# sMedX/FaceNet

Hardware: AMD Instinct MI355X
Metric: images/sec (160x160 triplet train) (higher is better)
Workload: dtype bf16

## Files before the change

facenet_amd/csrc/block_fused.hip:

```cpp
#include "common.h"
#include "../../include/facenet_hip.h"
#include <cstdlib>

namespace fn {

struct Block17Args {
    const unsigned short* x;
    unsigned short* y;
    const unsigned short* w_t0;
    const unsigned short* w_t1a;
    const unsigned short* w_t1b;
    const unsigned short* w_t1c;
    const unsigned short* w_up;
    const float* b_t0;
    const float* b_t1a;
    const float* b_t1b;
    const float* b_t1c;
    const float* b_up;
    float scale;
    int relu;
    int N;
    const unsigned char* warm;
    long warm_bytes;
};

enum { WARM_WGS = 64 };
__device__ __forceinline__ void warm_range(const unsigned char* p, long bytes, int j, int nthreads) {
    const long per = ((bytes + 8 * 16 - 1) / (8 * 16)) * 16;
    const long lo = (long)(j >> 3) * per, hi = lo + per < bytes ? lo + per : bytes;
    unsigned acc = 0u;
    for (long o = lo + (long)threadIdx.x * 16; o + 16 <= hi; o += (long)nthreads * 16 * 4) {
        u32x4 v[4];
#pragma unroll
        for (int u = 0; u < 4; ++u) {
            const long oo = o + (long)u * nthreads * 16;
            v[u] = oo + 16 <= hi ? *reinterpret_cast<const u32x4*>(p + oo) : u32x4{0u, 0u, 0u, 0u};
        }
#pragma unroll
        for (int u = 0; u < 4; ++u) acc ^= v[u][0];
    }
    asm volatile("" ::"v"(acc));
}

__device__ __forceinline__ int swz64(int row, int chunk) { return row * 64 + ((chunk ^ (((row >> 2) & 1) << 1)) << 4); }

#define FN_RING_PIPELINE(D_, NT_, LOAD, STORE, COMPUTE)                                   \
    {                                                                                       \
        _Pragma("unroll") for (int d_ = 0; d_ < (D_); ++d_) { LOAD(min(d_, (NT_) - 1), d_) } \
        STORE(0, 0)                                                                         \
        LOAD(min((D_), (NT_) - 1), 0)                                                       \
        __syncthreads();                                                                    \
        for (int kt0_ = 0; kt0_ < (NT_); kt0_ += (D_)) {                                    \
            _Pragma("unroll") for (int d_ = 0; d_ < (D_); ++d_) {                           \
                const int kt_ = kt0_ + d_;                                                  \
                if (kt_ < (NT_)) {                                                          \
                    STORE((d_ + 1) & 1, (d_ + 1) % (D_))                                    \
                    LOAD(min(kt_ + 1 + (D_), (NT_) - 1), (d_ + 1) % (D_))                   \
                    COMPUTE(kt_, d_ & 1, d_)                                                \
                    __syncthreads();                                                        \
                }                                                                           \
            }                                                                               \
        }                                                                                   \
    }

#define FN_DMA_PIPELINE(U_, NT_, ISSUE, COMPUTE)                                          \
    {                                                                                       \
        ISSUE(0, 0)                                                                         \
        ISSUE(min(1, (NT_) - 1), 1)                                                         \
        for (int kt0_ = 0; kt0_ < (NT_); kt0_ += (U_)) {                                    \
            _Pragma("unroll") for (int d_ = 0; d_ < (U_); ++d_) {                           \
                const int kt_ = kt0_ + d_;                                                  \
                if (kt_ < (NT_)) {                                                          \
                    asm volatile("s_waitcnt vmcnt(2)" ::: "memory");    \
                    __builtin_amdgcn_s_barrier();                       \
                    ISSUE(min(kt_ + 2, (NT_) - 1), (d_ + 2) % 3)                            \
                    COMPUTE(kt_, d_ % 3, d_)                                                \
                }                                                                           \
            }                                                                               \
        }                                                                                   \
        asm volatile("s_waitcnt vmcnt(0)" ::: "memory");                                    \
        __builtin_amdgcn_s_barrier();                                                       \
    }

template <typename T, bool DMA>
__global__ __launch_bounds__(512) void block17_infer_kernel(const Block17Args a) {
    constexpr int C = 896, CT = 128, NPIX = 64, D = 4;
    constexpr int DMA_BUF = 16 * 1024;
    typedef __attribute__((address_space(3))) void* lds_ptr;
    constexpr int PATCH_PIX = 112;
    constexpr int MIXED_BYTES = 8 * NPIX * 64;
    constexpr int PATCH_BYTES = 4 * PATCH_PIX * 64;
    constexpr int STAGE_BYTES = 20 * 1024;
    typedef typename LP<T>::vec8 vec8;

    extern __shared__ __attribute__((aligned(16))) unsigned char smem[];
    unsigned char* sMixed = smem;
    unsigned char* sT1a = sMixed + MIXED_BYTES;
    unsigned char* sT1b = sT1a + PATCH_BYTES;
    unsigned char* sStage = sT1b + PATCH_BYTES;
    float* sC = reinterpret_cast<float*>(sT1a);

    const int tid = threadIdx.x, lane = tid & 63, wave = tid >> 6, wq = wave & 3, wh = wave >> 2;
    const int fr = lane & 15, fq = lane >> 4;
    const int img = blockIdx.x;
    if (img >= a.N) {
        warm_range(a.warm, a.warm_bytes, img - a.N, 512);
        return;
    }
    const unsigned short* xin = a.x + (long)img * NPIX * C;
    const __amdgpu_buffer_rsrc_t rs_x = __builtin_amdgcn_make_buffer_rsrc(const_cast<unsigned short*>(xin), 0, NPIX * C * 2, 0x00020000);

    for (int i = tid; i < 2 * PATCH_BYTES / 16; i += 512) reinterpret_cast<u32x4*>(sT1a)[i] = u32x4{0u, 0u, 0u, 0u};

    {
        const int lrow = tid >> 2, lch = tid & 3;
        const __amdgpu_buffer_rsrc_t rs_w0 = __builtin_amdgcn_make_buffer_rsrc(const_cast<unsigned short*>(a.w_t0), 0, CT * C * 2, 0x00020000);
        const __amdgpu_buffer_rsrc_t rs_w1 = __builtin_amdgcn_make_buffer_rsrc(const_cast<unsigned short*>(a.w_t1a), 0, CT * C * 2, 0x00020000);
        f32x4 acc[2][4];
#pragma unroll
        for (int i = 0; i < 2; ++i)
#pragma unroll
            for (int j = 0; j < 4; ++j) acc[i][j] = f32x4{0.f, 0.f, 0.f, 0.f};
        u32x4 ra[D], rb[D][2];
        const int voff = (lrow * C + lch * 8) * 2;
        const int voff_x = ((lrow & 63) * C + lch * 8) * 2;
        const int st_a = swz64(lrow & 63, lch);
        int st_b[2], fa_off[2], fb_off[4];
#pragma unroll
        for (int q = 0; q < 2; ++q) st_b[q] = 4096 + swz64(lrow + 128 * q, lch);
#pragma unroll
        for (int i = 0; i < 2; ++i) fa_off[i] = swz64(wh * 32 + i * 16 + fr, fq);
#pragma unroll
        for (int j = 0; j < 4; ++j) fb_off[j] = 4096 + swz64(wq * 64 + j * 16 + fr, fq);
#define S1_LOAD(kt, d)                                                                                    \
        ra[d] = __builtin_amdgcn_raw_buffer_load_b128(rs_x, voff_x, (kt) * 64, 0);                         \
        rb[d][0] = __builtin_amdgcn_raw_buffer_load_b128(rs_w0, voff, (kt) * 64, 0);                       \
        rb[d][1] = __builtin_amdgcn_raw_buffer_load_b128(rs_w1, voff, (kt) * 64, 0);
#define S1_STORE(buf, d)                                                                                   \
        if (wh == 0) *reinterpret_cast<u32x4*>(sStage + (buf) * STAGE_BYTES + st_a) = ra[d];                 \
        _Pragma("unroll") for (int q = 0; q < 2; ++q) *reinterpret_cast<u32x4*>(sStage + (buf) * STAGE_BYTES + st_b[q]) = rb[d][q];
#define S1_COMPUTE(kt, buf, d)                                                                                           \
        {                                                                                                                  \
            vec8 fa[2], fb[4];                                                                                             \
            _Pragma("unroll") for (int i = 0; i < 2; ++i) fa[i] = *reinterpret_cast<const vec8*>(sStage + (buf) * STAGE_BYTES + fa_off[i]); \
            _Pragma("unroll") for (int j = 0; j < 4; ++j) fb[j] = *reinterpret_cast<const vec8*>(sStage + (buf) * STAGE_BYTES + fb_off[j]); \
            _Pragma("unroll") for (int i = 0; i < 2; ++i)                                                                  \
                _Pragma("unroll") for (int j = 0; j < 4; ++j) acc[i][j] = LP<T>::mfma(fa[i], fb[j], acc[i][j]);            \
        }
        FN_RING_PIPELINE(D, C / 32, S1_LOAD, S1_STORE, S1_COMPUTE)
#undef S1_LOAD
#undef S1_STORE
#undef S1_COMPUTE
#pragma unroll
        for (int j = 0; j < 4; ++j) {
            const int col = (wq & 1) * 64 + j * 16 + fr;
            const float bias = wq < 2 ? a.b_t0[col] : a.b_t1a[col];
            const int slice = col >> 5, cc = col & 31;
#pragma unroll
            for (int i = 0; i < 2; ++i)
#pragma unroll
                for (int r = 0; r < 4; ++r) {
                    const int p = wh * 32 + i * 16 + fq * 4 + r;
                    const unsigned short h = LP<T>::from_f32(fmaxf(acc[i][j][r] + bias, 0.f));
                    if (wq < 2) {
                        *reinterpret_cast<unsigned short*>(sMixed + slice * (NPIX * 64) + swz64(p, cc >> 3) + (cc & 7) * 2) = h;
                    } else {
                        const int pidx = (p >> 3) * 14 + (p & 7) + 3;
                        *reinterpret_cast<unsigned short*>(sT1a + slice * (PATCH_PIX * 64) + swz64(pidx, cc >> 3) + (cc & 7) * 2) = h;
                    }
                }
        }
        __syncthreads();
    }

    const int srow = tid >> 3, sch = tid & 7;
    int sl_off[2], fb_off[2][2];
#pragma unroll
    for (int q = 0; q < 2; ++q) sl_off[q] = (srow + 64 * q) * 128 + ((sch ^ ((srow + 64 * q) & 7)) << 4);
#pragma unroll
    for (int h = 0; h < 2; ++h)
#pragma unroll
        for (int j = 0; j < 2; ++j) {
            const int rw = wq * 32 + j * 16 + fr;
            fb_off[h][j] = rw * 128 + (((h * 4 + fq) ^ (rw & 7)) << 4);
        }
#define SLAB_STORE(buf, d) \
        _Pragma("unroll") for (int q = 0; q < 2; ++q) *reinterpret_cast<u32x4*>(sStage + (buf) * STAGE_BYTES + sl_off[q]) = rb[d][q];

#pragma unroll 1
    for (int stage = 2; stage <= 3; ++stage) {
        const unsigned short* wgt = stage == 2 ? a.w_t1b : a.w_t1c;
        const __amdgpu_buffer_rsrc_t rs_w = __builtin_amdgcn_make_buffer_rsrc(const_cast<unsigned short*>(wgt), 0, CT * 7 * CT * 2, 0x00020000);
        const float* bias_p = stage == 2 ? a.b_t1b : a.b_t1c;
        const unsigned char* src = stage == 2 ? sT1a : sT1b;
        const int tstep = stage == 2 ? 1 : 8;
        f32x4 acc[2][2];
#pragma unroll
        for (int i = 0; i < 2; ++i)
#pragma unroll
            for (int j = 0; j < 2; ++j) acc[i][j] = f32x4{0.f, 0.f, 0.f, 0.f};
        int fa_off[7][2];
#pragma unroll
        for (int t = 0; t < 7; ++t)
#pragma unroll
            for (int i = 0; i < 2; ++i) {
                const int p = wh * 32 + i * 16 + fr;
                const int base = stage == 2 ? (p >> 3) * 14 + (p & 7) : p;
                fa_off[t][i] = swz64(base + t * tstep, fq);
            }
        u32x4 rb[D][2];
        const int voff = (srow * (7 * CT) + sch * 8) * 2;
#define S23_LOAD(kt, d)                                                                                                         \
        _Pragma("unroll") for (int q = 0; q < 2; ++q)                                                                            \
            rb[d][q] = __builtin_amdgcn_raw_buffer_load_b128(rs_w, voff + 64 * q * (7 * CT) * 2, (((kt) >> 1) * CT + ((kt) & 1) * 64) * 2, 0);
#define S23_TAP(TAP, buf, half)                                                                                                  \
        _Pragma("unroll") for (int h = 0; h < 2; ++h) {                                                                          \
            vec8 fa[2], fb[2];                                                                                                   \
            _Pragma("unroll") for (int i = 0; i < 2; ++i)                                                                        \
                fa[i] = *reinterpret_cast<const vec8*>(src + ((half) * 2 + h) * (PATCH_PIX * 64) + fa_off[TAP][i]);              \
            _Pragma("unroll") for (int j = 0; j < 2; ++j) fb[j] = *reinterpret_cast<const vec8*>(sStage + (buf) * STAGE_BYTES + fb_off[h][j]); \
            _Pragma("unroll") for (int i = 0; i < 2; ++i)                                                                        \
                _Pragma("unroll") for (int j = 0; j < 2; ++j) acc[i][j] = LP<T>::mfma(fa[i], fb[j], acc[i][j]);                  \
        }
#define S23_COMPUTE(kt, buf, d)                                                                                                  \
        {                                                                                                                        \
            const int g = (kt) >> 2;                             \
            if ((d) < 2) {                                                                                                       \
                if (g == 0) { S23_TAP(0, buf, (d) & 1) } else if (g == 1) { S23_TAP(2, buf, (d) & 1) }                           \
                else if (g == 2) { S23_TAP(4, buf, (d) & 1) } else { S23_TAP(6, buf, (d) & 1) }                                  \
            } else {                                                                                                             \
                if (g == 0) { S23_TAP(1, buf, (d) & 1) } else if (g == 1) { S23_TAP(3, buf, (d) & 1) } else { S23_TAP(5, buf, (d) & 1) } \
            }                                                                                                                    \
        }
        if constexpr (DMA) {
#define S23_DMA_ISSUE(kt, buf)                                                                                               \
            _Pragma("unroll") for (int q = 0; q < 2; ++q)                                                                        \
                __builtin_amdgcn_raw_ptr_buffer_load_lds(rs_w, (lds_ptr)(sStage + (buf) * DMA_BUF + (wave * 16 + 8 * q) * 128), 16,   \
                                                         dma_voff23[q], (((kt) >> 1) * CT + ((kt) & 1) * 64) * 2, 0, 0);
#define S23_DMA_FB(buf, h, j) *reinterpret_cast<const vec8*>(sStage + (buf) * DMA_BUF + fb_off[h][j])
#define S23_DMA_TAP(TAP, buf, half)                                                                                              \
            _Pragma("unroll") for (int h = 0; h < 2; ++h) {                                                                      \
                vec8 fa[2], fb[2];                                                                                               \
                _Pragma("unroll") for (int i = 0; i < 2; ++i)                                                                    \
                    fa[i] = *reinterpret_cast<const vec8*>(src + ((half) * 2 + h) * (PATCH_PIX * 64) + fa_off[TAP][i]);          \
                _Pragma("unroll") for (int j = 0; j < 2; ++j) fb[j] = S23_DMA_FB(buf, h, j);                                     \
                _Pragma("unroll") for (int i = 0; i < 2; ++i)                                                                    \
                    _Pragma("unroll") for (int j = 0; j < 2; ++j) acc[i][j] = LP<T>::mfma(fa[i], fb[j], acc[i][j]);              \
            }
#define S23_DMA_COMPUTE(kt, buf, d)                                                                                              \
            {                                                                                                                    \
                const int g = (kt) / 6;                                                                             \
                if (((d) >> 1) == 0) { if (g == 0) { S23_DMA_TAP(0, buf, (d) & 1) } else if (g == 1) { S23_DMA_TAP(3, buf, (d) & 1) } else { S23_DMA_TAP(6, buf, (d) & 1) } } \
                else if (((d) >> 1) == 1) { if (g == 0) { S23_DMA_TAP(1, buf, (d) & 1) } else { S23_DMA_TAP(4, buf, (d) & 1) } } \
                else { if (g == 0) { S23_DMA_TAP(2, buf, (d) & 1) } else { S23_DMA_TAP(5, buf, (d) & 1) } }                      \
            }
            int dma_voff23[2];
#pragma unroll
            for (int q = 0; q < 2; ++q) {
                const int r = wave * 16 + 8 * q + (lane >> 3), cs = (lane & 7) ^ (r & 7);
                dma_voff23[q] = (r * (7 * CT) + cs * 8) * 2;
            }
            FN_DMA_PIPELINE(6, 14, S23_DMA_ISSUE, S23_DMA_COMPUTE)
#undef S23_DMA_ISSUE
#undef S23_DMA_FB
#undef S23_DMA_TAP
#undef S23_DMA_COMPUTE
        } else {
            FN_RING_PIPELINE(D, 14, S23_LOAD, SLAB_STORE, S23_COMPUTE)
        }
#undef S23_LOAD
#undef S23_TAP
#undef S23_COMPUTE
#pragma unroll
        for (int j = 0; j < 2; ++j) {
            const int col = wq * 32 + j * 16 + fr;
            const float bias = bias_p[col];
            const int slice = col >> 5, cc = col & 31;
#pragma unroll
            for (int i = 0; i < 2; ++i)
#pragma unroll
                for (int r = 0; r < 4; ++r) {
                    const int p = wh * 32 + i * 16 + fq * 4 + r;
                    const unsigned short h = LP<T>::from_f32(fmaxf(acc[i][j][r] + bias, 0.f));
                    if (stage == 2) *reinterpret_cast<unsigned short*>(sT1b + slice * (PATCH_PIX * 64) + swz64(p + 24, cc >> 3) + (cc & 7) * 2) = h;
                    else *reinterpret_cast<unsigned short*>(sMixed + (4 + slice) * (NPIX * 64) + swz64(p, cc >> 3) + (cc & 7) * 2) = h;
                }
        }
        __syncthreads();
    }

    {
        constexpr int CLD = 132;
        const __amdgpu_buffer_rsrc_t rs_w = __builtin_amdgcn_make_buffer_rsrc(const_cast<unsigned short*>(a.w_up), 0, C * 256 * 2, 0x00020000);
        u32x4 rb[D][2];
        const int voff = (srow * 256 + sch * 8) * 2;
        int fa_off[2];
#pragma unroll
        for (int i = 0; i < 2; ++i) fa_off[i] = swz64(wh * 32 + i * 16 + fr, fq);
        f32x4 acc[2][2];
#define S4_LOAD(kt, d)                                                                                                           \
        _Pragma("unroll") for (int q = 0; q < 2; ++q)                                                                            \
            rb[d][q] = __builtin_amdgcn_raw_buffer_load_b128(rs_w, voff + 64 * q * 256 * 2, ((((kt) >> 2) * 128) * 256 + ((kt) & 3) * 64) * 2, 0);
#define S4_COMPUTE(kt, buf, d)                                                                                                   \
        {                                                                                                                        \
            if ((d) == 0) {                                                                                                      \
                _Pragma("unroll") for (int i = 0; i < 2; ++i)                                                                    \
                    _Pragma("unroll") for (int j = 0; j < 2; ++j) acc[i][j] = f32x4{0.f, 0.f, 0.f, 0.f};                         \
            }                                                                                                                    \
            _Pragma("unroll") for (int h = 0; h < 2; ++h) {                                                                      \
                vec8 fa[2], fb[2];                                                                                               \
                _Pragma("unroll") for (int i = 0; i < 2; ++i)                                                                    \
                    fa[i] = *reinterpret_cast<const vec8*>(sMixed + ((d) * 2 + h) * (NPIX * 64) + fa_off[i]);                    \
                _Pragma("unroll") for (int j = 0; j < 2; ++j) fb[j] = *reinterpret_cast<const vec8*>(sStage + (buf) * STAGE_BYTES + fb_off[h][j]); \
                _Pragma("unroll") for (int i = 0; i < 2; ++i)                                                                    \
                    _Pragma("unroll") for (int j = 0; j < 2; ++j) acc[i][j] = LP<T>::mfma(fa[i], fb[j], acc[i][j]);              \
            }                                                                                                                    \
            if ((d) == 3) {                 \
                const int pass = (kt) >> 2;                                                                                      \
                _Pragma("unroll") for (int i = 0; i < 2; ++i)                                                                    \
                    _Pragma("unroll") for (int j = 0; j < 2; ++j)                                                                \
                        _Pragma("unroll") for (int r = 0; r < 4; ++r)                                                            \
                            sC[(wh * 32 + i * 16 + fq * 4 + r) * CLD + wq * 32 + j * 16 + fr] = acc[i][j][r];                            \
                __syncthreads();                                                                                                 \
                _Pragma("unroll") for (int q = 0; q < 2; ++q) {              \
                    const int idx = tid + 512 * q, p = idx >> 4, cg = idx & 15;                                                  \
                    const int col = pass * 128 + cg * 8;                                                                         \
                    const f32x4 c0 = *reinterpret_cast<const f32x4*>(&sC[p * CLD + cg * 8]);                                     \
                    const f32x4 c1 = *reinterpret_cast<const f32x4*>(&sC[p * CLD + cg * 8 + 4]);                                 \
                    const f32x4 b0 = *reinterpret_cast<const f32x4*>(a.b_up + col), b1 = *reinterpret_cast<const f32x4*>(a.b_up + col + 4); \
                    float rv[8], v[8];                                                                                           \
                    unpack8<T>(load_global_b128(xin, (long)p * C + col), rv);                                                    \
                    _Pragma("unroll") for (int e = 0; e < 4; ++e) {                                                              \
                        v[e] = rv[e] + a.scale * (c0[e] + b0[e]);                                                                \
                        v[4 + e] = rv[4 + e] + a.scale * (c1[e] + b1[e]);                                                        \
                    }                                                                                                            \
                    if (a.relu) {                                                                                                \
                        _Pragma("unroll") for (int e = 0; e < 8; ++e) v[e] = fmaxf(v[e], 0.f);                                   \
                    }                                                                                                            \
                    *reinterpret_cast<u32x4*>(a.y + ((long)img * NPIX + p) * C + col) = pack8<T>(v);                             \
                }                                                                                                                \
            }                                                                                                                    \
        }
        if constexpr (DMA) {
            int dma_voff4[2];
#pragma unroll
            for (int q = 0; q < 2; ++q) {
                const int r = wave * 16 + 8 * q + (lane >> 3), cs = (lane & 7) ^ (r & 7);
                dma_voff4[q] = (r * 256 + cs * 8) * 2;
            }
#define S4_DMA_ISSUE(kt, buf)                                                                                                    \
            _Pragma("unroll") for (int q = 0; q < 2; ++q)                                                                        \
                __builtin_amdgcn_raw_ptr_buffer_load_lds(rs_w, (lds_ptr)(sStage + (buf) * DMA_BUF + (wave * 16 + 8 * q) * 128), 16,   \
                                                         dma_voff4[q], ((((kt) >> 2) * 128) * 256 + ((kt) & 3) * 64) * 2, 0, 0);
#define S4_DMA_COMPUTE(kt, buf, d)                                                                                               \
            {                                                                                                                    \
                if (((d) & 3) == 0) {                                                                                            \
                    _Pragma("unroll") for (int i = 0; i < 2; ++i)                                                                \
                        _Pragma("unroll") for (int j = 0; j < 2; ++j) acc[i][j] = f32x4{0.f, 0.f, 0.f, 0.f};                     \
                }                                                                                                                \
                _Pragma("unroll") for (int h = 0; h < 2; ++h) {                                                                  \
                    vec8 fa[2], fb[2];                                                                                           \
                    _Pragma("unroll") for (int i = 0; i < 2; ++i)                                                                \
                        fa[i] = *reinterpret_cast<const vec8*>(sMixed + (((d) & 3) * 2 + h) * (NPIX * 64) + fa_off[i]);          \
                    _Pragma("unroll") for (int j = 0; j < 2; ++j) fb[j] = *reinterpret_cast<const vec8*>(sStage + (buf) * DMA_BUF + fb_off[h][j]); \
                    _Pragma("unroll") for (int i = 0; i < 2; ++i)                                                                \
                        _Pragma("unroll") for (int j = 0; j < 2; ++j) acc[i][j] = LP<T>::mfma(fa[i], fb[j], acc[i][j]);          \
                }                                                                                                                \
                if (((d) & 3) == 3) {                                                                                            \
                    const int pass = (kt) >> 2;                                                                                  \
                    _Pragma("unroll") for (int i = 0; i < 2; ++i)                                                                \
                        _Pragma("unroll") for (int j = 0; j < 2; ++j)                                                            \
                            _Pragma("unroll") for (int r = 0; r < 4; ++r)                                                        \
                                sC[(wh * 32 + i * 16 + fq * 4 + r) * CLD + wq * 32 + j * 16 + fr] = acc[i][j][r];                \
                    asm volatile("s_waitcnt lgkmcnt(0)" ::: "memory");                                                           \
                    __builtin_amdgcn_s_barrier();                                                                                \
                    _Pragma("unroll") for (int q = 0; q < 2; ++q) {                                                              \
                        const int idx = tid + 512 * q, p = idx >> 4, cg = idx & 15;                                              \
                        const int col = pass * 128 + cg * 8;                                                                     \
                        const f32x4 c0 = *reinterpret_cast<const f32x4*>(&sC[p * CLD + cg * 8]);                                 \
                        const f32x4 c1 = *reinterpret_cast<const f32x4*>(&sC[p * CLD + cg * 8 + 4]);                             \
                        const f32x4 b0 = *reinterpret_cast<const f32x4*>(a.b_up + col), b1 = *reinterpret_cast<const f32x4*>(a.b_up + col + 4); \
                        float rv[8], v[8];                                                                                       \
                        unpack8<T>(load_global_b128(xin, (long)p * C + col), rv);                                                \
                        _Pragma("unroll") for (int e = 0; e < 4; ++e) {                                                          \
                            v[e] = rv[e] + a.scale * (c0[e] + b0[e]);                                                            \
                            v[4 + e] = rv[4 + e] + a.scale * (c1[e] + b1[e]);                                                    \
                        }                                                                                                        \
                        if (a.relu) {                                                                                            \
                            _Pragma("unroll") for (int e = 0; e < 8; ++e) v[e] = fmaxf(v[e], 0.f);                               \
                        }                                                                                                        \
                        *reinterpret_cast<u32x4*>(a.y + ((long)img * NPIX + p) * C + col) = pack8<T>(v);                         \
                    }                                                                                                            \
                }                                                                                                                \
            }
            FN_DMA_PIPELINE(12, 28, S4_DMA_ISSUE, S4_DMA_COMPUTE)
#undef S4_DMA_ISSUE
#undef S4_DMA_COMPUTE
        } else {
            FN_RING_PIPELINE(D, 28, S4_LOAD, SLAB_STORE, S4_COMPUTE)
        }
#undef S4_LOAD
#undef S4_COMPUTE
    }
#undef SLAB_STORE
}

struct Block35Args {
    const unsigned short* x;
    unsigned short* y;
    const unsigned short* w_1x1[3];
    const unsigned short* w_3x3[3];
    const unsigned short* w_up;
    const float* b_1x1[3];
    const float* b_3x3[3];
    const float* b_up;
    float scale;
    int relu;
    int N;
    const unsigned char* warm;
    long warm_bytes;
};

template <typename T>
__global__ __launch_bounds__(512) void block35_infer_kernel(const Block35Args a) {
    constexpr int C = 256, NPIX = 289, MROWS = 304, D = 4;
    constexpr int SLICE_BYTES = MROWS * 64;
    constexpr int PATCH_PIX = 19 * 19, PATCH_BYTES = (PATCH_PIX * 64 + 1023) / 1024 * 1024 + 1024;
    constexpr int MIXED_BYTES = 3 * SLICE_BYTES;
    constexpr int STAGE_BYTES = SLICE_BYTES + 96 * 64;
    typedef typename LP<T>::vec8 vec8;

    extern __shared__ __attribute__((aligned(16))) unsigned char smem[];
    unsigned char* sMixed = smem;
    unsigned char* sP1 = sMixed + MIXED_BYTES;
    unsigned char* sP2 = sP1 + PATCH_BYTES;
    unsigned char* sStage = sP2 + PATCH_BYTES;
    float* sC = reinterpret_cast<float*>(sP1);

    const int tid = threadIdx.x, lane = tid & 63, wave = tid >> 6;
    const int fr = lane & 15, fq = lane >> 4;
    const int img = blockIdx.x;
    if (img >= a.N) {
        warm_range(a.warm, a.warm_bytes, img - a.N, 512);
        return;
    }
    const unsigned short* xin = a.x + (long)img * NPIX * C;
    const __amdgpu_buffer_rsrc_t rs_x = __builtin_amdgcn_make_buffer_rsrc(const_cast<unsigned short*>(xin), 0, NPIX * C * 2, 0x00020000);
    constexpr unsigned OOB = 0x60000000u;

    for (int i = tid; i < 2 * PATCH_BYTES / 16; i += 512) reinterpret_cast<u32x4*>(sP1)[i] = u32x4{0u, 0u, 0u, 0u};

    const int nfr = wave < 3 ? 3 : 2;
    int prow[3];
#pragma unroll
    for (int i = 0; i < 3; ++i) prow[i] = (wave + 8 * i) * 16 + fr;

    auto stage_weights = [&](unsigned char* dst, const unsigned short* w, int rows, int gstride, int goff) {
        for (int i = tid; i < rows * 4; i += 512) {
            const int r = i >> 2, ch = i & 3;
            *reinterpret_cast<u32x4*>(dst + swz64(r, ch)) = load_global_b128(w, (long)r * gstride + goff + ch * 8);
        }
    };
    auto store_frag = [&](const f32x4& v, float bias, unsigned char* region, int frag, int col, bool patch) {
        const int cc = col & 31;
#pragma unroll
        for (int r = 0; r < 4; ++r) {
            const int p = frag * 16 + fq * 4 + r;
            if (p < NPIX) {
                const int y = p / 17, x = p - y * 17;
                const int pidx = patch ? (y + 1) * 19 + x + 1 : p;
                *reinterpret_cast<unsigned short*>(region + swz64(pidx, cc >> 3) + (cc & 7) * 2) = LP<T>::from_f32(fmaxf(v[r] + bias, 0.f));
            }
        }
    };

    {
        f32x4 acc[3][6];
#pragma unroll
        for (int i = 0; i < 3; ++i)
#pragma unroll
            for (int j = 0; j < 6; ++j) acc[i][j] = f32x4{0.f, 0.f, 0.f, 0.f};
        u32x4 ra[D][3], rb[D];
        int voff_a[3], st_a[3];
#pragma unroll
        for (int q = 0; q < 3; ++q) {
            const int idx = tid + 512 * q, p = idx >> 2, ch = idx & 3;
            voff_a[q] = p < NPIX ? (p * C + ch * 8) * 2 : (int)OOB;
            st_a[q] = p < MROWS ? swz64(p, ch) : -1;
        }
        const int wr = tid >> 2, wch = tid & 3;
        const unsigned short* wrow = a.w_1x1[min(wr >> 5, 2)] + (long)(wr & 31) * C + wch * 8;
        const int st_b = wr < 96 ? SLICE_BYTES + swz64(wr, wch) : -1;
#define S1_LOAD(kt, d)                                                                                     \
        _Pragma("unroll") for (int q = 0; q < 3; ++q) ra[d][q] = __builtin_amdgcn_raw_buffer_load_b128(rs_x, voff_a[q], (kt) * 64, 0); \
        rb[d] = load_global_b128(wrow, (kt) * 32);
#define S1_STORE(buf, d)                                                                                   \
        _Pragma("unroll") for (int q = 0; q < 3; ++q)                                                        \
            if (st_a[q] >= 0) *reinterpret_cast<u32x4*>(sStage + (buf) * STAGE_BYTES + st_a[q]) = ra[d][q];  \
        if (st_b >= 0) *reinterpret_cast<u32x4*>(sStage + (buf) * STAGE_BYTES + st_b) = rb[d];
#define S1_COMPUTE(kt, buf, d)                                                                                           \
        {                                                                                                                  \
            const unsigned char* pa = sStage + (buf) * STAGE_BYTES;                                                        \
            vec8 fb[6];                                                                                                    \
            _Pragma("unroll") for (int j = 0; j < 6; ++j) fb[j] = *reinterpret_cast<const vec8*>(pa + SLICE_BYTES + swz64(j * 16 + fr, fq)); \
            _Pragma("unroll") for (int i = 0; i < 3; ++i)                                                                  \
                if (i < nfr) {                                                                                             \
                    const vec8 fa = *reinterpret_cast<const vec8*>(pa + swz64(prow[i], fq));                               \
                    _Pragma("unroll") for (int j = 0; j < 6; ++j) acc[i][j] = LP<T>::mfma(fa, fb[j], acc[i][j]);           \
                }                                                                                                          \
        }
        FN_RING_PIPELINE(D, C / 32, S1_LOAD, S1_STORE, S1_COMPUTE)
#undef S1_LOAD
#undef S1_STORE
#undef S1_COMPUTE
#pragma unroll
        for (int j = 0; j < 6; ++j) {
            const int col = j * 16 + fr, t = col >> 5;
            const float bias = a.b_1x1[t][col & 31];
            unsigned char* region = t == 0 ? sMixed : (t == 1 ? sP1 : sP2);
#pragma unroll
            for (int i = 0; i < 3; ++i)
                if (i < nfr) store_frag(acc[i][j], bias, region, wave + 8 * i, col, t != 0);
        }
        __syncthreads();
    }

    int fa_tap[9][3];
#pragma unroll
    for (int t = 0; t < 9; ++t)
#pragma unroll
        for (int i = 0; i < 3; ++i) {
            const int p = min(prow[i], NPIX - 1);
            const int y = p / 17, x = p - y * 17;
            fa_tap[t][i] = swz64((y + t / 3) * 19 + x + t % 3, fq);
        }
#pragma unroll 1
    for (int c3 = 0; c3 < 3; ++c3) {
        const unsigned char* src = c3 == 1 ? sP2 : sP1;
        for (int i = tid; i < 9 * 32 * 4; i += 512) {
            const int r = i >> 2, ch = i & 3, tap = r >> 5, co = r & 31;
            *reinterpret_cast<u32x4*>(sStage + swz64(r, ch)) = load_global_b128(a.w_3x3[c3], (long)co * 288 + tap * 32 + ch * 8);
        }
        __syncthreads();
        f32x4 acc[3][2];
#pragma unroll
        for (int i = 0; i < 3; ++i)
#pragma unroll
            for (int j = 0; j < 2; ++j) acc[i][j] = f32x4{0.f, 0.f, 0.f, 0.f};
#pragma unroll
        for (int t = 0; t < 9; ++t) {
            vec8 fb[2];
#pragma unroll
            for (int j = 0; j < 2; ++j) fb[j] = *reinterpret_cast<const vec8*>(sStage + swz64(t * 32 + j * 16 + fr, fq));
#pragma unroll
            for (int i = 0; i < 3; ++i)
                if (i < nfr) {
                    const vec8 fa = *reinterpret_cast<const vec8*>(src + fa_tap[t][i]);
#pragma unroll
                    for (int j = 0; j < 2; ++j) acc[i][j] = LP<T>::mfma(fa, fb[j], acc[i][j]);
                }
        }
        __syncthreads();
#pragma unroll
        for (int j = 0; j < 2; ++j) {
            const int col = j * 16 + fr;
            const float bias = a.b_3x3[c3][col];
            unsigned char* region = c3 == 0 ? sMixed + SLICE_BYTES : (c3 == 1 ? sP1 : sMixed + 2 * SLICE_BYTES);
#pragma unroll
            for (int i = 0; i < 3; ++i)
                if (i < nfr) store_frag(acc[i][j], bias, region, wave + 8 * i, col, c3 == 1);
        }
        __syncthreads();
    }

    {
        constexpr int CLD = 36;
        for (int i = tid; i < 3 * 256 * 4; i += 512) {
            const int r = i >> 2, ch = i & 3, sl = r >> 8, co = r & 255;
            *reinterpret_cast<u32x4*>(sStage + swz64(r, ch)) = load_global_b128(a.w_up, (long)co * 96 + sl * 32 + ch * 8);
        }
        __syncthreads();
#pragma unroll 1
        for (int pass = 0; pass < 8; ++pass) {
            f32x4 acc[3][2];
#pragma unroll
            for (int i = 0; i < 3; ++i)
#pragma unroll
                for (int j = 0; j < 2; ++j) acc[i][j] = f32x4{0.f, 0.f, 0.f, 0.f};
#pragma unroll
            for (int sl = 0; sl < 3; ++sl) {
                vec8 fb[2];
#pragma unroll
                for (int j = 0; j < 2; ++j) fb[j] = *reinterpret_cast<const vec8*>(sStage + swz64(sl * 256 + pass * 32 + j * 16 + fr, fq));
#pragma unroll
                for (int i = 0; i < 3; ++i)
                    if (i < nfr) {
                        const vec8 fa = *reinterpret_cast<const vec8*>(sMixed + sl * SLICE_BYTES + swz64(prow[i], fq));
#pragma unroll
                        for (int j = 0; j < 2; ++j) acc[i][j] = LP<T>::mfma(fa, fb[j], acc[i][j]);
                    }
            }
#pragma unroll
            for (int i = 0; i < 3; ++i)
                if (i < nfr) {
#pragma unroll
                    for (int j = 0; j < 2; ++j)
#pragma unroll
                        for (int r = 0; r < 4; ++r) sC[((wave + 8 * i) * 16 + fq * 4 + r) * CLD + j * 16 + fr] = acc[i][j][r];
                }
            __syncthreads();
            for (int idx = tid; idx < NPIX * 4; idx += 512) {
                const int p = idx >> 2, cg = idx & 3;
                const int col = pass * 32 + cg * 8;
                const f32x4 c0 = *reinterpret_cast<const f32x4*>(&sC[p * CLD + cg * 8]);
                const f32x4 c1 = *reinterpret_cast<const f32x4*>(&sC[p * CLD + cg * 8 + 4]);
                const f32x4 b0 = *reinterpret_cast<const f32x4*>(a.b_up + col), b1 = *reinterpret_cast<const f32x4*>(a.b_up + col + 4);
                float rv[8], v[8];
                unpack8<T>(load_global_b128(xin, (long)p * C + col), rv);
#pragma unroll
                for (int e = 0; e < 4; ++e) {
                    v[e] = rv[e] + a.scale * (c0[e] + b0[e]);
                    v[4 + e] = rv[4 + e] + a.scale * (c1[e] + b1[e]);
                }
                if (a.relu) {
#pragma unroll
                    for (int e = 0; e < 8; ++e) v[e] = fmaxf(v[e], 0.f);
                }
                *reinterpret_cast<u32x4*>(a.y + ((long)img * NPIX + p) * C + col) = pack8<T>(v);
            }
            __syncthreads();
        }
    }
}

}

using namespace fn;

extern "C" int fn_block17_infer(const void* x, void* y, int N, const void* w_t0, const void* w_t1a, const void* w_t1b, const void* w_t1c,
                                const void* w_up, const float* b_t0, const float* b_t1a, const float* b_t1b, const float* b_t1c, const float* b_up,
                                float scale, int relu, int dtype, void* stream) {
    return fn_block17_infer_warm(x, y, N, w_t0, w_t1a, w_t1b, w_t1c, w_up, b_t0, b_t1a, b_t1b, b_t1c, b_up, scale, relu, nullptr, 0, dtype, stream);
}

extern "C" int fn_block17_infer_warm(const void* x, void* y, int N, const void* w_t0, const void* w_t1a, const void* w_t1b, const void* w_t1c,
                                     const void* w_up, const float* b_t0, const float* b_t1a, const float* b_t1b, const float* b_t1c,
                                     const float* b_up, float scale, int relu, const void* warm, int64_t warm_bytes, int dtype, void* stream) {
    FN_REQUIRE(dtype == FN_BF16 || dtype == FN_F16, "dtype %d unsupported", dtype);
    FN_REQUIRE((warm == nullptr) == (warm_bytes == 0) && warm_bytes >= 0 && warm_bytes < (1L << 31) && ((uintptr_t)warm & 15) == 0,
               "block17_infer: warm range must be 16-byte aligned, below 2 GiB, and given with its size");
    FN_REQUIRE(x && y && x != y && N > 0 && w_t0 && w_t1a && w_t1b && w_t1c && w_up && b_t0 && b_t1a && b_t1b && b_t1c && b_up,
               "block17_infer: bad arguments");
    Block17Args a{(const unsigned short*)x, (unsigned short*)y, (const unsigned short*)w_t0, (const unsigned short*)w_t1a,
                  (const unsigned short*)w_t1b, (const unsigned short*)w_t1c, (const unsigned short*)w_up, b_t0, b_t1a, b_t1b, b_t1c, b_up,
                  scale, relu, N, (const unsigned char*)warm, (long)warm_bytes};
    const int grid = N + (warm ? WARM_WGS : 0);
    constexpr size_t smem = 8 * 64 * 64 + 2 * 4 * 112 * 64 + 3 * 16 * 1024;
    static const int use_dma = env_int("FN_B17_DMA", 1);
    static LdsOptIn ok[4];
    const void* kerns[4] = {reinterpret_cast<const void*>(block17_infer_kernel<__bf16, false>), reinterpret_cast<const void*>(block17_infer_kernel<_Float16, false>),
                            reinterpret_cast<const void*>(block17_infer_kernel<__bf16, true>), reinterpret_cast<const void*>(block17_infer_kernel<_Float16, true>)};
    const int which = (use_dma ? 2 : 0) + (dtype == FN_BF16 ? 0 : 1);
    if (int rc = allow_big_lds(kerns[which], ok[which], "block17_infer")) return rc;
    if (use_dma) {
        if (dtype == FN_BF16) hipLaunchKernelGGL((block17_infer_kernel<__bf16, true>), dim3(grid), dim3(512), smem, (hipStream_t)stream, a);
        else hipLaunchKernelGGL((block17_infer_kernel<_Float16, true>), dim3(grid), dim3(512), smem, (hipStream_t)stream, a);
    } else {
        if (dtype == FN_BF16) hipLaunchKernelGGL((block17_infer_kernel<__bf16, false>), dim3(grid), dim3(512), smem, (hipStream_t)stream, a);
        else hipLaunchKernelGGL((block17_infer_kernel<_Float16, false>), dim3(grid), dim3(512), smem, (hipStream_t)stream, a);
    }
    return check_launch("block17_infer");
}

extern "C" int fn_block35_infer(const void* x, void* y, int N, const void* const* w_1x1, const void* const* w_3x3, const void* w_up,
                                const float* const* b_1x1, const float* const* b_3x3, const float* b_up, float scale, int relu, int dtype,
                                void* stream) {
    return fn_block35_infer_warm(x, y, N, w_1x1, w_3x3, w_up, b_1x1, b_3x3, b_up, scale, relu, nullptr, 0, dtype, stream);
}

extern "C" int fn_block35_infer_warm(const void* x, void* y, int N, const void* const* w_1x1, const void* const* w_3x3, const void* w_up,
                                     const float* const* b_1x1, const float* const* b_3x3, const float* b_up, float scale, int relu,
                                     const void* warm, int64_t warm_bytes, int dtype, void* stream) {
    FN_REQUIRE(dtype == FN_BF16 || dtype == FN_F16, "dtype %d unsupported", dtype);
    FN_REQUIRE((warm == nullptr) == (warm_bytes == 0) && warm_bytes >= 0 && warm_bytes < (1L << 31) && ((uintptr_t)warm & 15) == 0,
               "block35_infer: warm range must be 16-byte aligned, below 2 GiB, and given with its size");
    FN_REQUIRE(x && y && x != y && N > 0 && w_1x1 && w_3x3 && w_up && b_1x1 && b_3x3 && b_up, "block35_infer: bad arguments");
    Block35Args a{};
    a.x = (const unsigned short*)x; a.y = (unsigned short*)y; a.w_up = (const unsigned short*)w_up; a.b_up = b_up;
    for (int i = 0; i < 3; ++i) {
        FN_REQUIRE(w_1x1[i] && w_3x3[i] && b_1x1[i] && b_3x3[i], "block35_infer: null layer %d", i);
        a.w_1x1[i] = (const unsigned short*)w_1x1[i]; a.w_3x3[i] = (const unsigned short*)w_3x3[i];
        a.b_1x1[i] = b_1x1[i]; a.b_3x3[i] = b_3x3[i];
    }
    a.scale = scale; a.relu = relu; a.N = N;
    a.warm = (const unsigned char*)warm; a.warm_bytes = (long)warm_bytes;
    const int grid = N + (warm ? WARM_WGS : 0);
    constexpr int SLICE = 304 * 64, PATCH = (19 * 19 * 64 + 1023) / 1024 * 1024 + 1024;
    constexpr size_t smem = 3 * SLICE + 2 * PATCH + 2 * (SLICE + 96 * 64);
    static_assert(smem <= 160 * 1024 && 3 * 256 * 64 <= 2 * (SLICE + 96 * 64) && 304 * 36 * 4 <= 2 * PATCH, "block35 LDS plan");
    static LdsOptIn ok[2];
    const int which = dtype == FN_BF16 ? 0 : 1;
    if (int rc = allow_big_lds(which == 0 ? reinterpret_cast<const void*>(block35_infer_kernel<__bf16>) : reinterpret_cast<const void*>(block35_infer_kernel<_Float16>),
                               ok[which], "block35_infer")) return rc;
    if (dtype == FN_BF16) hipLaunchKernelGGL(block35_infer_kernel<__bf16>, dim3(grid), dim3(512), smem, (hipStream_t)stream, a);
    else hipLaunchKernelGGL(block35_infer_kernel<_Float16>, dim3(grid), dim3(512), smem, (hipStream_t)stream, a);
    return check_launch("block35_infer");
}
```

Baseline: 13950.

## Add DMA path for block17 stage 1, vectorize epilogues, prefetch residuals

Stage 1 of the fused block17 kernel gets a direct-to-LDS buffer-load DMA pipeline that replaces the register ring. The DMA pipeline macro now takes a group size and a per-step wait. MFMA operands are swapped so each lane holds four consecutive output columns, which lets the epilogues add bias, apply ReLU and store packed 8-byte LDS writes instead of scalar 2-byte stores. Biases are loaded once up front. The final up-projection stage prefetches residual and bias for the next pass with double buffering. Optional timing instrumentation is added behind a compile flag, and LDS staging grows to 60 KB.

New measurement: 14180, median of 6. 1.6% higher.

```diff
diff --git a/facenet_amd/csrc/block_fused.hip b/facenet_amd/csrc/block_fused.hip
--- a/facenet_amd/csrc/block_fused.hip
+++ b/facenet_amd/csrc/block_fused.hip
@@ -1,6 +1,44 @@
 #include "common.h"
 #include "../../include/facenet_hip.h"
 #include <cstdlib>
+
+#ifndef FN_FUSED_PHASES
+#define FN_FUSED_PHASES 0
+#endif
+
+#if FN_FUSED_PHASES
+__device__ unsigned long long fn_fused_phase[256 * 2 * 32];
+extern "C" int fn_debug_fused_phases(unsigned long long* out, int reset) {
+    static unsigned long long host[256 * 2 * 32];
+    if (out) {
+        if (hipMemcpyFromSymbol(host, HIP_SYMBOL(fn_fused_phase), sizeof(host)) != hipSuccess) return -1;
+        for (int i = 0; i < 2 * 32; ++i) {
+            out[i] = 0;
+            for (int r = 0; r < 256; ++r) out[i] += host[r * 2 * 32 + i];
+        }
+    }
+    if (reset) {
+        for (auto& v : host) v = 0;
+        if (hipMemcpyToSymbol(HIP_SYMBOL(fn_fused_phase), host, sizeof(host)) != hipSuccess) return -1;
+    }
+    return 0;
+}
+#define FN_PH_INIT(kern)                                                                                  \
+    unsigned long long* const ph_p = fn_fused_phase + ((blockIdx.x & 255) * 2 + (kern)) * 32;            \
+    unsigned long long ph_last = wall_clock64();                                                          \
+    if (threadIdx.x == 0) atomicAdd(ph_p, 1ull);
+#define FN_PH(slot)                                                                                       \
+    {                                                                                                     \
+        const unsigned long long ph_t = wall_clock64();                                                   \
+        if (threadIdx.x == 0) atomicAdd(ph_p + (slot), ph_t - ph_last);                                   \
+        ph_last = ph_t;                                                                                   \
+    }
+#define FN_PH_WAIT(n) asm volatile("s_waitcnt vmcnt(" #n ")" ::: "memory");
+#else
+#define FN_PH_INIT(kern)
+#define FN_PH(slot)
+#define FN_PH_WAIT(n)
+#endif
 
 namespace fn {
 
@@ -44,6 +82,15 @@
 
 __device__ __forceinline__ int swz64(int row, int chunk) { return row * 64 + ((chunk ^ (((row >> 2) & 1) << 1)) << 4); }
 
+typedef __attribute__((ext_vector_type(2))) unsigned int u32x2;
+template <typename T> __device__ __forceinline__ u32x2 pack4_bias_relu(const f32x4& v, const f32x4& b) {
+    u32x2 o;
+    o[0] = (unsigned)LP<T>::from_f32(fmaxf(v[0] + b[0], 0.f)) | ((unsigned)LP<T>::from_f32(fmaxf(v[1] + b[1], 0.f)) << 16);
+    o[1] = (unsigned)LP<T>::from_f32(fmaxf(v[2] + b[2], 0.f)) | ((unsigned)LP<T>::from_f32(fmaxf(v[3] + b[3], 0.f)) << 16);
+    return o;
+}
+__device__ __forceinline__ f32x4 load_bias4(const float* b) { return f32x4{b[0], b[1], b[2], b[3]}; }
+
 #define FN_RING_PIPELINE(D_, NT_, LOAD, STORE, COMPUTE)                                   \
     {                                                                                       \
         _Pragma("unroll") for (int d_ = 0; d_ < (D_); ++d_) { LOAD(min(d_, (NT_) - 1), d_) } \
@@ -63,18 +110,22 @@
         }                                                                                   \
     }
 
-#define FN_DMA_PIPELINE(U_, NT_, ISSUE, COMPUTE)                                          \
+#define FN_DMA_WAIT2(d) asm volatile("s_waitcnt vmcnt(2)" ::: "memory");
+#define FN_DMA_PIPELINE(U_, G_, NT_, WAIT, ISSUE, COMPUTE)                                \
     {                                                                                       \
+        static_assert((U_) % (G_) == 0 && (NT_) % (G_) == 0 && (U_) % 3 == 0, "DMA pipeline shape"); \
         ISSUE(0, 0)                                                                         \
         ISSUE(min(1, (NT_) - 1), 1)                                                         \
         for (int kt0_ = 0; kt0_ < (NT_); kt0_ += (U_)) {                                    \
-            _Pragma("unroll") for (int d_ = 0; d_ < (U_); ++d_) {                           \
-                const int kt_ = kt0_ + d_;                                                  \
-                if (kt_ < (NT_)) {                                                          \
-                    asm volatile("s_waitcnt vmcnt(2)" ::: "memory");    \
-                    __builtin_amdgcn_s_barrier();                       \
-                    ISSUE(min(kt_ + 2, (NT_) - 1), (d_ + 2) % 3)                            \
-                    COMPUTE(kt_, d_ % 3, d_)                                                \
+            _Pragma("unroll") for (int g_ = 0; g_ < (U_) / (G_); ++g_) {                    \
+                if (kt0_ + g_ * (G_) < (NT_)) {                                             \
+                    _Pragma("unroll") for (int e_ = 0; e_ < (G_); ++e_) {                   \
+                        const int d_ = g_ * (G_) + e_, kt_ = kt0_ + d_;                     \
+                        WAIT(d_)                                            \
+                        __builtin_amdgcn_s_barrier();                       \
+                        ISSUE(min(kt_ + 2, (NT_) - 1), (d_ + 2) % 3)                        \
+                        COMPUTE(kt_, d_ % 3, d_)                                            \
+                    }                                                                       \
                 }                                                                           \
             }                                                                               \
         }                                                                                   \
@@ -107,6 +158,7 @@
         warm_range(a.warm, a.warm_bytes, img - a.N, 512);
         return;
     }
+    FN_PH_INIT(0)
     const unsigned short* xin = a.x + (long)img * NPIX * C;
     const __amdgpu_buffer_rsrc_t rs_x = __builtin_amdgcn_make_buffer_rsrc(const_cast<unsigned short*>(xin), 0, NPIX * C * 2, 0x00020000);
 
@@ -121,6 +173,10 @@
         for (int i = 0; i < 2; ++i)
 #pragma unroll
             for (int j = 0; j < 4; ++j) acc[i][j] = f32x4{0.f, 0.f, 0.f, 0.f};
+        f32x4 bias[4];
+#pragma unroll
+        for (int j = 0; j < 4; ++j) bias[j] = load_bias4((wq < 2 ? a.b_t0 : a.b_t1a) + (wq & 1) * 64 + j * 16 + fq * 4);
+        FN_PH(1)
         u32x4 ra[D], rb[D][2];
         const int voff = (lrow * C + lch * 8) * 2;
         const int voff_x = ((lrow & 63) * C + lch * 8) * 2;
@@ -145,32 +201,44 @@
             _Pragma("unroll") for (int i = 0; i < 2; ++i) fa[i] = *reinterpret_cast<const vec8*>(sStage + (buf) * STAGE_BYTES + fa_off[i]); \
             _Pragma("unroll") for (int j = 0; j < 4; ++j) fb[j] = *reinterpret_cast<const vec8*>(sStage + (buf) * STAGE_BYTES + fb_off[j]); \
             _Pragma("unroll") for (int i = 0; i < 2; ++i)                                                                  \
-                _Pragma("unroll") for (int j = 0; j < 4; ++j) acc[i][j] = LP<T>::mfma(fa[i], fb[j], acc[i][j]);            \
-        }
-        FN_RING_PIPELINE(D, C / 32, S1_LOAD, S1_STORE, S1_COMPUTE)
+                _Pragma("unroll") for (int j = 0; j < 4; ++j) acc[i][j] = LP<T>::mfma(fb[j], fa[i], acc[i][j]);            \
+        }
+        if constexpr (DMA) {
+            const int wv = __builtin_amdgcn_readfirstlane(wave);
+            const int drow = lane >> 2, dchunk = (lane & 3) ^ (((lane >> 4) & 1) << 1);
+            const __amdgpu_buffer_rsrc_t rs_wd = wv < 4 ? rs_w0 : rs_w1;
+            const int dma_voff_w = (((wv & 3) * 32 + drow) * C + dchunk * 8) * 2, dma_voff_x = ((wv * 16 + drow) * C + dchunk * 8) * 2;
+#define S1_DMA_WAIT(d)                                                                                                    \
+            if (wv < 4) { asm volatile("s_waitcnt vmcnt(3)" ::: "memory"); } else { asm volatile("s_waitcnt vmcnt(2)" ::: "memory"); }
+#define S1_DMA_ISSUE(kt, buf)                                                                                             \
+            _Pragma("unroll") for (int q = 0; q < 2; ++q)                                                                  \
+                __builtin_amdgcn_raw_ptr_buffer_load_lds(rs_wd, (lds_ptr)(sStage + (buf) * STAGE_BYTES + 4096 + (wv * 2 + q) * 1024), 16, \
+                                                         dma_voff_w + q * 16 * C * 2, (kt) * 64, 0, 0);                    \
+            if (wv < 4)                                                                                                  \
+                __builtin_amdgcn_raw_ptr_buffer_load_lds(rs_x, (lds_ptr)(sStage + (buf) * STAGE_BYTES + wv * 1024), 16, dma_voff_x, (kt) * 64, 0, 0);
+            FN_DMA_PIPELINE(12, 4, C / 32, S1_DMA_WAIT, S1_DMA_ISSUE, S1_COMPUTE)
+#undef S1_DMA_WAIT
+#undef S1_DMA_ISSUE
+        } else {
+            FN_RING_PIPELINE(D, C / 32, S1_LOAD, S1_STORE, S1_COMPUTE)
+        }
 #undef S1_LOAD
 #undef S1_STORE
 #undef S1_COMPUTE
+        FN_PH(2)
 #pragma unroll
         for (int j = 0; j < 4; ++j) {
-            const int col = (wq & 1) * 64 + j * 16 + fr;
-            const float bias = wq < 2 ? a.b_t0[col] : a.b_t1a[col];
-            const int slice = col >> 5, cc = col & 31;
-#pragma unroll
-            for (int i = 0; i < 2; ++i)
-#pragma unroll
-                for (int r = 0; r < 4; ++r) {
-                    const int p = wh * 32 + i * 16 + fq * 4 + r;
-                    const unsigned short h = LP<T>::from_f32(fmaxf(acc[i][j][r] + bias, 0.f));
-                    if (wq < 2) {
-                        *reinterpret_cast<unsigned short*>(sMixed + slice * (NPIX * 64) + swz64(p, cc >> 3) + (cc & 7) * 2) = h;
-                    } else {
-                        const int pidx = (p >> 3) * 14 + (p & 7) + 3;
-                        *reinterpret_cast<unsigned short*>(sT1a + slice * (PATCH_PIX * 64) + swz64(pidx, cc >> 3) + (cc & 7) * 2) = h;
-                    }
-                }
+            const int slice = (wq & 1) * 2 + (j >> 1), sub = ((j & 1) * 2 + (fq >> 1)), byte = (fq & 1) * 8;
+#pragma unroll
+            for (int i = 0; i < 2; ++i) {
+                const int p = wh * 32 + i * 16 + fr;
+                const u32x2 h = pack4_bias_relu<T>(acc[i][j], bias[j]);
+                if (wq < 2) *reinterpret_cast<u32x2*>(sMixed + slice * (NPIX * 64) + swz64(p, sub) + byte) = h;
+                else *reinterpret_cast<u32x2*>(sT1a + slice * (PATCH_PIX * 64) + swz64((p >> 3) * 14 + (p & 7) + 3, sub) + byte) = h;
+            }
         }
         __syncthreads();
+        FN_PH(3)
     }
 
     const int srow = tid >> 3, sch = tid & 7;
@@ -208,6 +276,9 @@
                 const int base = stage == 2 ? (p >> 3) * 14 + (p & 7) : p;
                 fa_off[t][i] = swz64(base + t * tstep, fq);
             }
+        f32x4 bias[2];
+#pragma unroll
+        for (int j = 0; j < 2; ++j) bias[j] = load_bias4(bias_p + wq * 32 + j * 16 + fq * 4);
         u32x4 rb[D][2];
         const int voff = (srow * (7 * CT) + sch * 8) * 2;
 #define S23_LOAD(kt, d)                                                                                                         \
@@ -220,7 +291,7 @@
                 fa[i] = *reinterpret_cast<const vec8*>(src + ((half) * 2 + h) * (PATCH_PIX * 64) + fa_off[TAP][i]);              \
             _Pragma("unroll") for (int j = 0; j < 2; ++j) fb[j] = *reinterpret_cast<const vec8*>(sStage + (buf) * STAGE_BYTES + fb_off[h][j]); \
             _Pragma("unroll") for (int i = 0; i < 2; ++i)                                                                        \
-                _Pragma("unroll") for (int j = 0; j < 2; ++j) acc[i][j] = LP<T>::mfma(fa[i], fb[j], acc[i][j]);                  \
+                _Pragma("unroll") for (int j = 0; j < 2; ++j) acc[i][j] = LP<T>::mfma(fb[j], fa[i], acc[i][j]);                  \
         }
 #define S23_COMPUTE(kt, buf, d)                                                                                                  \
         {                                                                                                                        \
@@ -245,7 +316,7 @@
                     fa[i] = *reinterpret_cast<const vec8*>(src + ((half) * 2 + h) * (PATCH_PIX * 64) + fa_off[TAP][i]);          \
                 _Pragma("unroll") for (int j = 0; j < 2; ++j) fb[j] = S23_DMA_FB(buf, h, j);                                     \
                 _Pragma("unroll") for (int i = 0; i < 2; ++i)                                                                    \
-                    _Pragma("unroll") for (int j = 0; j < 2; ++j) acc[i][j] = LP<T>::mfma(fa[i], fb[j], acc[i][j]);              \
+                    _Pragma("unroll") for (int j = 0; j < 2; ++j) acc[i][j] = LP<T>::mfma(fb[j], fa[i], acc[i][j]);              \
             }
 #define S23_DMA_COMPUTE(kt, buf, d)                                                                                              \
             {                                                                                                                    \
@@ -260,7 +331,7 @@
                 const int r = wave * 16 + 8 * q + (lane >> 3), cs = (lane & 7) ^ (r & 7);
                 dma_voff23[q] = (r * (7 * CT) + cs * 8) * 2;
             }
-            FN_DMA_PIPELINE(6, 14, S23_DMA_ISSUE, S23_DMA_COMPUTE)
+            FN_DMA_PIPELINE(6, 2, 14, FN_DMA_WAIT2, S23_DMA_ISSUE, S23_DMA_COMPUTE)
 #undef S23_DMA_ISSUE
 #undef S23_DMA_FB
 #undef S23_DMA_TAP
@@ -271,22 +342,20 @@
 #undef S23_LOAD
 #undef S23_TAP
 #undef S23_COMPUTE
+        FN_PH(stage * 2)
 #pragma unroll
         for (int j = 0; j < 2; ++j) {
-            const int col = wq * 32 + j * 16 + fr;
-            const float bias = bias_p[col];
-            const int slice = col >> 5, cc = col & 31;
-#pragma unroll
-            for (int i = 0; i < 2; ++i)
-#pragma unroll
-                for (int r = 0; r < 4; ++r) {
-                    const int p = wh * 32 + i * 16 + fq * 4 + r;
-                    const unsigned short h = LP<T>::from_f32(fmaxf(acc[i][j][r] + bias, 0.f));
-                    if (stage == 2) *reinterpret_cast<unsigned short*>(sT1b + slice * (PATCH_PIX * 64) + swz64(p + 24, cc >> 3) + (cc & 7) * 2) = h;
-                    else *reinterpret_cast<unsigned short*>(sMixed + (4 + slice) * (NPIX * 64) + swz64(p, cc >> 3) + (cc & 7) * 2) = h;
-                }
+            const int sub = j * 2 + (fq >> 1), byte = (fq & 1) * 8;
+#pragma unroll
+            for (int i = 0; i < 2; ++i) {
+                const int p = wh * 32 + i * 16 + fr;
+                const u32x2 h = pack4_bias_relu<T>(acc[i][j], bias[j]);
+                if (stage == 2) *reinterpret_cast<u32x2*>(sT1b + wq * (PATCH_PIX * 64) + swz64(p + 24, sub) + byte) = h;
+                else *reinterpret_cast<u32x2*>(sMixed + (4 + wq) * (NPIX * 64) + swz64(p, sub) + byte) = h;
+            }
         }
         __syncthreads();
+        FN_PH(stage * 2 + 1)
     }
 
     {
@@ -298,48 +367,59 @@
 #pragma unroll
         for (int i = 0; i < 2; ++i) fa_off[i] = swz64(wh * 32 + i * 16 + fr, fq);
         f32x4 acc[2][2];
-#define S4_LOAD(kt, d)                                                                                                           \
-        _Pragma("unroll") for (int q = 0; q < 2; ++q)                                                                            \
-            rb[d][q] = __builtin_amdgcn_raw_buffer_load_b128(rs_w, voff + 64 * q * 256 * 2, ((((kt) >> 2) * 128) * 256 + ((kt) & 3) * 64) * 2, 0);
-#define S4_COMPUTE(kt, buf, d)                                                                                                   \
+        const int ep_p = tid >> 4, ep_cg = tid & 15;
+        const int voff_res = (ep_p * C + ep_cg * 8) * 2;
+        u32x4 rres[2];
+        f32x4 bup[2];
+#define S4_PREFETCH(pass)                                                                                                        \
         {                                                                                                                        \
-            if ((d) == 0) {                                                                                                      \
+            _Pragma("unroll") for (int q = 0; q < 2; ++q)                                                                        \
+                rres[q] = __builtin_amdgcn_raw_buffer_load_b128(rs_x, voff_res + q * 32 * C * 2, (pass) * 128 * 2, 0);           \
+            bup[0] = *reinterpret_cast<const f32x4*>(a.b_up + (pass) * 128 + ep_cg * 8);                                         \
+            bup[1] = *reinterpret_cast<const f32x4*>(a.b_up + (pass) * 128 + ep_cg * 8 + 4);                                     \
+        }
+#define S4_MULTIPLY(kk, SLAB)                                                                                                    \
+        {                                                                                                                        \
+            if ((kk) == 0) {                                                                                                     \
                 _Pragma("unroll") for (int i = 0; i < 2; ++i)                                                                    \
                     _Pragma("unroll") for (int j = 0; j < 2; ++j) acc[i][j] = f32x4{0.f, 0.f, 0.f, 0.f};                         \
             }                                                                                                                    \
             _Pragma("unroll") for (int h = 0; h < 2; ++h) {                                                                      \
                 vec8 fa[2], fb[2];                                                                                               \
                 _Pragma("unroll") for (int i = 0; i < 2; ++i)                                                                    \
-                    fa[i] = *reinterpret_cast<const vec8*>(sMixed + ((d) * 2 + h) * (NPIX * 64) + fa_off[i]);                    \
-                _Pragma("unroll") for (int j = 0; j < 2; ++j) fb[j] = *reinterpret_cast<const vec8*>(sStage + (buf) * STAGE_BYTES + fb_off[h][j]); \
+                    fa[i] = *reinterpret_cast<const vec8*>(sMixed + ((kk) * 2 + h) * (NPIX * 64) + fa_off[i]);                   \
+                _Pragma("unroll") for (int j = 0; j < 2; ++j) fb[j] = *reinterpret_cast<const vec8*>((SLAB) + fb_off[h][j]);     \
                 _Pragma("unroll") for (int i = 0; i < 2; ++i)                                                                    \
-                    _Pragma("unroll") for (int j = 0; j < 2; ++j) acc[i][j] = LP<T>::mfma(fa[i], fb[j], acc[i][j]);              \
+                    _Pragma("unroll") for (int j = 0; j < 2; ++j) acc[i][j] = LP<T>::mfma(fb[j], fa[i], acc[i][j]);              \
             }                                                                                                                    \
-            if ((d) == 3) {                 \
-                const int pass = (kt) >> 2;                                                                                      \
-                _Pragma("unroll") for (int i = 0; i < 2; ++i)                                                                    \
-                    _Pragma("unroll") for (int j = 0; j < 2; ++j)                                                                \
-                        _Pragma("unroll") for (int r = 0; r < 4; ++r)                                                            \
-                            sC[(wh * 32 + i * 16 + fq * 4 + r) * CLD + wq * 32 + j * 16 + fr] = acc[i][j][r];                            \
-                __syncthreads();                                                                                                 \
-                _Pragma("unroll") for (int q = 0; q < 2; ++q) {              \
-                    const int idx = tid + 512 * q, p = idx >> 4, cg = idx & 15;                                                  \
-                    const int col = pass * 128 + cg * 8;                                                                         \
-                    const f32x4 c0 = *reinterpret_cast<const f32x4*>(&sC[p * CLD + cg * 8]);                                     \
-                    const f32x4 c1 = *reinterpret_cast<const f32x4*>(&sC[p * CLD + cg * 8 + 4]);                                 \
-                    const f32x4 b0 = *reinterpret_cast<const f32x4*>(a.b_up + col), b1 = *reinterpret_cast<const f32x4*>(a.b_up + col + 4); \
-                    float rv[8], v[8];                                                                                           \
-                    unpack8<T>(load_global_b128(xin, (long)p * C + col), rv);                                                    \
-                    _Pragma("unroll") for (int e = 0; e < 4; ++e) {                                                              \
-                        v[e] = rv[e] + a.scale * (c0[e] + b0[e]);                                                                \
-                        v[4 + e] = rv[4 + e] + a.scale * (c1[e] + b1[e]);                                                        \
-                    }                                                                                                            \
-                    if (a.relu) {                                                                                                \
-                        _Pragma("unroll") for (int e = 0; e < 8; ++e) v[e] = fmaxf(v[e], 0.f);                                   \
-                    }                                                                                                            \
-                    *reinterpret_cast<u32x4*>(a.y + ((long)img * NPIX + p) * C + col) = pack8<T>(v);                             \
+        }
+#define S4_PASS_EPILOGUE(pass, BARRIER)                                                                                          \
+        {                                                                                                                        \
+            FN_PH(8)                                                                                                             \
+            _Pragma("unroll") for (int i = 0; i < 2; ++i)                                                                        \
+                _Pragma("unroll") for (int j = 0; j < 2; ++j)                                                                    \
+                    *reinterpret_cast<f32x4*>(&sC[(wh * 32 + i * 16 + fr) * CLD + wq * 32 + j * 16 + fq * 4]) = acc[i][j];       \
+            BARRIER                                                                                                              \
+            FN_PH(9)                                                                                                             \
+            FN_PH_WAIT(8)                   \
+            FN_PH(10)                                                                                                            \
+            _Pragma("unroll") for (int q = 0; q < 2; ++q) {                                                                      \
+                const int pp = ep_p + 32 * q, col = (pass) * 128 + ep_cg * 8;                                                    \
+                const f32x4 c0 = *reinterpret_cast<const f32x4*>(&sC[pp * CLD + ep_cg * 8]);                                     \
+                const f32x4 c1 = *reinterpret_cast<const f32x4*>(&sC[pp * CLD + ep_cg * 8 + 4]);                                 \
+                const f32x4 b0 = bup[0], b1 = bup[1];                                                                            \
+                float rv[8], v[8];                                                                                               \
+                unpack8<T>(rres[q], rv);                                                                                         \
+                _Pragma("unroll") for (int e = 0; e < 4; ++e) {                                                                  \
+                    v[e] = rv[e] + a.scale * (c0[e] + b0[e]);                                                                    \
+                    v[4 + e] = rv[4 + e] + a.scale * (c1[e] + b1[e]);                                                            \
                 }                                                                                                                \
+                if (a.relu) {                                                                                                    \
+                    _Pragma("unroll") for (int e = 0; e < 8; ++e) v[e] = fmaxf(v[e], 0.f);                                       \
+                }                                                                                                                \
+                *reinterpret_cast<u32x4*>(a.y + ((long)img * NPIX + pp) * C + col) = pack8<T>(v);                                \
             }                                                                                                                    \
+            FN_PH(11)                                                                                                            \
         }
         if constexpr (DMA) {
             int dma_voff4[2];
@@ -348,59 +428,40 @@
                 const int r = wave * 16 + 8 * q + (lane >> 3), cs = (lane & 7) ^ (r & 7);
                 dma_voff4[q] = (r * 256 + cs * 8) * 2;
             }
+#define S4_DMA_WAIT(d)                                                                                                           \
+            if (((d) & 3) == 1) { asm volatile("s_waitcnt vmcnt(6)" ::: "memory"); } else { asm volatile("s_waitcnt vmcnt(2)" ::: "memory"); }
 #define S4_DMA_ISSUE(kt, buf)                                                                                                    \
             _Pragma("unroll") for (int q = 0; q < 2; ++q)                                                                        \
                 __builtin_amdgcn_raw_ptr_buffer_load_lds(rs_w, (lds_ptr)(sStage + (buf) * DMA_BUF + (wave * 16 + 8 * q) * 128), 16,   \
                                                          dma_voff4[q], ((((kt) >> 2) * 128) * 256 + ((kt) & 3) * 64) * 2, 0, 0);
 #define S4_DMA_COMPUTE(kt, buf, d)                                                                                               \
             {                                                                                                                    \
-                if (((d) & 3) == 0) {                                                                                            \
-                    _Pragma("unroll") for (int i = 0; i < 2; ++i)                                                                \
-                        _Pragma("unroll") for (int j = 0; j < 2; ++j) acc[i][j] = f32x4{0.f, 0.f, 0.f, 0.f};                     \
-                }                                                                                                                \
-                _Pragma("unroll") for (int h = 0; h < 2; ++h) {                                                                  \
-                    vec8 fa[2], fb[2];                                                                                           \
-                    _Pragma("unroll") for (int i = 0; i < 2; ++i)                                                                \
-                        fa[i] = *reinterpret_cast<const vec8*>(sMixed + (((d) & 3) * 2 + h) * (NPIX * 64) + fa_off[i]);          \
-                    _Pragma("unroll") for (int j = 0; j < 2; ++j) fb[j] = *reinterpret_cast<const vec8*>(sStage + (buf) * DMA_BUF + fb_off[h][j]); \
-                    _Pragma("unroll") for (int i = 0; i < 2; ++i)                                                                \
-                        _Pragma("unroll") for (int j = 0; j < 2; ++j) acc[i][j] = LP<T>::mfma(fa[i], fb[j], acc[i][j]);          \
-                }                                                                                                                \
-                if (((d) & 3) == 3) {                                                                                            \
-                    const int pass = (kt) >> 2;                                                                                  \
-                    _Pragma("unroll") for (int i = 0; i < 2; ++i)                                                                \
-                        _Pragma("unroll") for (int j = 0; j < 2; ++j)                                                            \
-                            _Pragma("unroll") for (int r = 0; r < 4; ++r)                                                        \
-                                sC[(wh * 32 + i * 16 + fq * 4 + r) * CLD + wq * 32 + j * 16 + fr] = acc[i][j][r];                \
-                    asm volatile("s_waitcnt lgkmcnt(0)" ::: "memory");                                                           \
-                    __builtin_amdgcn_s_barrier();                                                                                \
-                    _Pragma("unroll") for (int q = 0; q < 2; ++q) {                                                              \
-                        const int idx = tid + 512 * q, p = idx >> 4, cg = idx & 15;                                              \
-                        const int col = pass * 128 + cg * 8;                                                                     \
-                        const f32x4 c0 = *reinterpret_cast<const f32x4*>(&sC[p * CLD + cg * 8]);                                 \
-                        const f32x4 c1 = *reinterpret_cast<const f32x4*>(&sC[p * CLD + cg * 8 + 4]);                             \
-                        const f32x4 b0 = *reinterpret_cast<const f32x4*>(a.b_up + col), b1 = *reinterpret_cast<const f32x4*>(a.b_up + col + 4); \
-                        float rv[8], v[8];                                                                                       \
-                        unpack8<T>(load_global_b128(xin, (long)p * C + col), rv);                                                \
-                        _Pragma("unroll") for (int e = 0; e < 4; ++e) {                                                          \
-                            v[e] = rv[e] + a.scale * (c0[e] + b0[e]);                                                            \
-                            v[4 + e] = rv[4 + e] + a.scale * (c1[e] + b1[e]);                                                    \
-                        }                                                                                                        \
-                        if (a.relu) {                                                                                            \
-                            _Pragma("unroll") for (int e = 0; e < 8; ++e) v[e] = fmaxf(v[e], 0.f);                               \
-                        }                                                                                                        \
-                        *reinterpret_cast<u32x4*>(a.y + ((long)img * NPIX + p) * C + col) = pack8<T>(v);                         \
-                    }                                                                                                            \
-                }                                                                                                                \
-            }
-            FN_DMA_PIPELINE(12, 28, S4_DMA_ISSUE, S4_DMA_COMPUTE)
+                if (((d) & 3) == 0) S4_PREFETCH((kt) >> 2)                                                                       \
+                S4_MULTIPLY((d) & 3, sStage + (buf) * DMA_BUF)                                                                   \
+                if (((d) & 3) == 3)                                                                                              \
+                    S4_PASS_EPILOGUE((kt) >> 2, asm volatile("s_waitcnt lgkmcnt(0)" ::: "memory"); __builtin_amdgcn_s_barrier();) \
+            }
+            FN_DMA_PIPELINE(12, 4, 28, S4_DMA_WAIT, S4_DMA_ISSUE, S4_DMA_COMPUTE)
+#undef S4_DMA_WAIT
 #undef S4_DMA_ISSUE
 #undef S4_DMA_COMPUTE
         } else {
+#define S4_LOAD(kt, d)                                                                                                           \
+            _Pragma("unroll") for (int q = 0; q < 2; ++q)                                                                        \
+                rb[d][q] = __builtin_amdgcn_raw_buffer_load_b128(rs_w, voff + 64 * q * 256 * 2, ((((kt) >> 2) * 128) * 256 + ((kt) & 3) * 64) * 2, 0);
+#define S4_COMPUTE(kt, buf, d)                                                                                \
+            {                                                                                                                    \
+                if ((d) == 0) S4_PREFETCH((kt) >> 2)                                                                             \
+                S4_MULTIPLY(d, sStage + (buf) * STAGE_BYTES)                                                                     \
+                if ((d) == 3) S4_PASS_EPILOGUE((kt) >> 2, __syncthreads();)                                                      \
+            }
             FN_RING_PIPELINE(D, 28, S4_LOAD, SLAB_STORE, S4_COMPUTE)
-        }
 #undef S4_LOAD
 #undef S4_COMPUTE
+        }
+#undef S4_PREFETCH
+#undef S4_MULTIPLY
+#undef S4_PASS_EPILOGUE
     }
 #undef SLAB_STORE
 }
@@ -428,7 +489,9 @@
     constexpr int PATCH_PIX = 19 * 19, PATCH_BYTES = (PATCH_PIX * 64 + 1023) / 1024 * 1024 + 1024;
     constexpr int MIXED_BYTES = 3 * SLICE_BYTES;
     constexpr int STAGE_BYTES = SLICE_BYTES + 96 * 64;
+    static_assert(9 * 32 * 64 <= SLICE_BYTES && 3 * 256 * 64 <= 2 * STAGE_BYTES && MROWS * 36 * 4 <= 2 * PATCH_BYTES, "block35 LDS plan");
     typedef typename LP<T>::vec8 vec8;
+    typedef __attribute__((address_space(3))) void* lds_ptr;
 
     extern __shared__ __attribute__((aligned(16))) unsigned char smem[];
     unsigned char* sMixed = smem;
@@ -447,31 +510,44 @@
     const unsigned short* xin = a.x + (long)img * NPIX * C;
     const __amdgpu_buffer_rsrc_t rs_x = __builtin_amdgcn_make_buffer_rsrc(const_cast<unsigned short*>(xin), 0, NPIX * C * 2, 0x00020000);
     constexpr unsigned OOB = 0x60000000u;
+    FN_PH_INIT(1)
+
+    const int dma_row = lane >> 2, dma_chunk = (lane & 3) ^ (((lane >> 4) & 1) << 1);
+    auto dma_w3x3 = [&](unsigned char* dst, const unsigned short* w) {
+        const __amdgpu_buffer_rsrc_t rs = __builtin_amdgcn_make_buffer_rsrc(const_cast<unsigned short*>(w), 0, 32 * 288 * 2, 0x00020000);
+#pragma unroll
+        for (int k = 0; k < 3; ++k) {
+            const int n = wave + 8 * k;
+            if (n < 18) {
+                const int r = n * 16 + dma_row;
+                __builtin_amdgcn_raw_ptr_buffer_load_lds(rs, (lds_ptr)(dst + n * 1024), 16, ((r & 31) * 288 + (r >> 5) * 32 + dma_chunk * 8) * 2, 0, 0, 0);
+            }
+        }
+    };
+    auto dma_wup = [&](unsigned char* dst) {
+        const __amdgpu_buffer_rsrc_t rs = __builtin_amdgcn_make_buffer_rsrc(const_cast<unsigned short*>(a.w_up), 0, 256 * 96 * 2, 0x00020000);
+#pragma unroll
+        for (int k = 0; k < 6; ++k) {
+            const int n = wave + 8 * k, r = n * 16 + dma_row;
+            __builtin_amdgcn_raw_ptr_buffer_load_lds(rs, (lds_ptr)(dst + n * 1024), 16, ((r & 255) * 96 + (r >> 8) * 32 + dma_chunk * 8) * 2, 0, 0, 0);
+        }
+    };
+    unsigned char* const sW3 = sMixed + 2 * SLICE_BYTES;
+    dma_w3x3(sW3, a.w_3x3[0]);
 
     for (int i = tid; i < 2 * PATCH_BYTES / 16; i += 512) reinterpret_cast<u32x4*>(sP1)[i] = u32x4{0u, 0u, 0u, 0u};
 
     const int nfr = wave < 3 ? 3 : 2;
-    int prow[3];
-#pragma unroll
-    for (int i = 0; i < 3; ++i) prow[i] = (wave + 8 * i) * 16 + fr;
-
-    auto stage_weights = [&](unsigned char* dst, const unsigned short* w, int rows, int gstride, int goff) {
-        for (int i = tid; i < rows * 4; i += 512) {
-            const int r = i >> 2, ch = i & 3;
-            *reinterpret_cast<u32x4*>(dst + swz64(r, ch)) = load_global_b128(w, (long)r * gstride + goff + ch * 8);
-        }
-    };
-    auto store_frag = [&](const f32x4& v, float bias, unsigned char* region, int frag, int col, bool patch) {
-        const int cc = col & 31;
-#pragma unroll
-        for (int r = 0; r < 4; ++r) {
-            const int p = frag * 16 + fq * 4 + r;
-            if (p < NPIX) {
-                const int y = p / 17, x = p - y * 17;
-                const int pidx = patch ? (y + 1) * 19 + x + 1 : p;
-                *reinterpret_cast<unsigned short*>(region + swz64(pidx, cc >> 3) + (cc & 7) * 2) = LP<T>::from_f32(fmaxf(v[r] + bias, 0.f));
-            }
-        }
+    int prow[3], ppatch[3];
+#pragma unroll
+    for (int i = 0; i < 3; ++i) {
+        prow[i] = (wave + 8 * i) * 16 + fr;
+        const int y = prow[i] / 17, x = prow[i] - y * 17;
+        ppatch[i] = (y + 1) * 19 + x + 1;
+    }
+    auto store_frag = [&](const f32x4& v, const f32x4& bias, unsigned char* region, int i, int j, bool patch) {
+        if (prow[i] < NPIX)
+            *reinterpret_cast<u32x2*>(region + swz64(patch ? ppatch[i] : prow[i], (j & 1) * 2 + (fq >> 1)) + (fq & 1) * 8) = pack4_bias_relu<T>(v, bias);
     };
 
     {
@@ -491,6 +567,10 @@
         const int wr = tid >> 2, wch = tid & 3;
         const unsigned short* wrow = a.w_1x1[min(wr >> 5, 2)] + (long)(wr & 31) * C + wch * 8;
         const int st_b = wr < 96 ? SLICE_BYTES + swz64(wr, wch) : -1;
+        f32x4 bias[6];
+#pragma unroll
+        for (int j = 0; j < 6; ++j) bias[j] = load_bias4(a.b_1x1[j >> 1] + (j & 1) * 16 + fq * 4);
+        FN_PH(1)
 #define S1_LOAD(kt, d)                                                                                     \
         _Pragma("unroll") for (int q = 0; q < 3; ++q) ra[d][q] = __builtin_amdgcn_raw_buffer_load_b128(rs_x, voff_a[q], (kt) * 64, 0); \
         rb[d] = load_global_b128(wrow, (kt) * 32);
@@ -506,23 +586,24 @@
             _Pragma("unroll") for (int i = 0; i < 3; ++i)                                                                  \
                 if (i < nfr) {                                                                                             \
                     const vec8 fa = *reinterpret_cast<const vec8*>(pa + swz64(prow[i], fq));                               \
-                    _Pragma("unroll") for (int j = 0; j < 6; ++j) acc[i][j] = LP<T>::mfma(fa, fb[j], acc[i][j]);           \
+                    _Pragma("unroll") for (int j = 0; j < 6; ++j) acc[i][j] = LP<T>::mfma(fb[j], fa, acc[i][j]);           \
                 }                                                                                                          \
         }
         FN_RING_PIPELINE(D, C / 32, S1_LOAD, S1_STORE, S1_COMPUTE)
 #undef S1_LOAD
 #undef S1_STORE
 #undef S1_COMPUTE
+        FN_PH(2)
 #pragma unroll
         for (int j = 0; j < 6; ++j) {
-            const int col = j * 16 + fr, t = col >> 5;
-            const float bias = a.b_1x1[t][col & 31];
+            const int t = j >> 1;
             unsigned char* region = t == 0 ? sMixed : (t == 1 ? sP1 : sP2);
 #pragma unroll
             for (int i = 0; i < 3; ++i)
-                if (i < nfr) store_frag(acc[i][j], bias, region, wave + 8 * i, col, t != 0);
+                if (i < nfr) store_frag(acc[i][j], bias[j], region, i, j, t != 0);
         }
         __syncthreads();
+        FN_PH(3)
     }
 
     int fa_tap[9][3];
@@ -537,11 +618,14 @@
 #pragma unroll 1
     for (int c3 = 0; c3 < 3; ++c3) {
         const unsigned char* src = c3 == 1 ? sP2 : sP1;
-        for (int i = tid; i < 9 * 32 * 4; i += 512) {
-            const int r = i >> 2, ch = i & 3, tap = r >> 5, co = r & 31;
-            *reinterpret_cast<u32x4*>(sStage + swz64(r, ch)) = load_global_b128(a.w_3x3[c3], (long)co * 288 + tap * 32 + ch * 8);
-        }
-        __syncthreads();
+        const unsigned char* wsl = c3 == 1 ? sStage : sW3;
+        f32x4 bias[2];
+#pragma unroll
+        for (int j = 0; j < 2; ++j) bias[j] = load_bias4(a.b_3x3[c3] + j * 16 + fq * 4);
+        if (c3 == 0) dma_w3x3(sStage, a.w_3x3[1]);
+        else if (c3 == 1) dma_w3x3(sW3, a.w_3x3[2]);
+        else dma_wup(sStage);
+        FN_PH(4 + 3 * c3)
         f32x4 acc[3][2];
 #pragma unroll
         for (int i = 0; i < 3; ++i)
@@ -551,85 +635,96 @@
         for (int t = 0; t < 9; ++t) {
             vec8 fb[2];
 #pragma unroll
-            for (int j = 0; j < 2; ++j) fb[j] = *reinterpret_cast<const vec8*>(sStage + swz64(t * 32 + j * 16 + fr, fq));
+            for (int j = 0; j < 2; ++j) fb[j] = *reinterpret_cast<const vec8*>(wsl + swz64(t * 32 + j * 16 + fr, fq));
 #pragma unroll
             for (int i = 0; i < 3; ++i)
                 if (i < nfr) {
                     const vec8 fa = *reinterpret_cast<const vec8*>(src + fa_tap[t][i]);
 #pragma unroll
-                    for (int j = 0; j < 2; ++j) acc[i][j] = LP<T>::mfma(fa, fb[j], acc[i][j]);
+                    for (int j = 0; j < 2; ++j) acc[i][j] = LP<T>::mfma(fb[j], fa, acc[i][j]);
                 }
         }
         __syncthreads();
-#pragma unroll
-        for (int j = 0; j < 2; ++j) {
-            const int col = j * 16 + fr;
-            const float bias = a.b_3x3[c3][col];
-            unsigned char* region = c3 == 0 ? sMixed + SLICE_BYTES : (c3 == 1 ? sP1 : sMixed + 2 * SLICE_BYTES);
+        FN_PH(5 + 3 * c3)
+        unsigned char* region = c3 == 0 ? sMixed + SLICE_BYTES : (c3 == 1 ? sP1 : sMixed + 2 * SLICE_BYTES);
+#pragma unroll
+        for (int j = 0; j < 2; ++j)
 #pragma unroll
             for (int i = 0; i < 3; ++i)
-                if (i < nfr) store_frag(acc[i][j], bias, region, wave + 8 * i, col, c3 == 1);
-        }
+                if (i < nfr) store_frag(acc[i][j], bias[j], region, i, j, c3 == 1);
+        asm volatile("s_waitcnt vmcnt(0)" ::: "memory");
         __syncthreads();
+        FN_PH(6 + 3 * c3)
     }
 
     {
         constexpr int CLD = 36;
-        for (int i = tid; i < 3 * 256 * 4; i += 512) {
-            const int r = i >> 2, ch = i & 3, sl = r >> 8, co = r & 255;
-            *reinterpret_cast<u32x4*>(sStage + swz64(r, ch)) = load_global_b128(a.w_up, (long)co * 96 + sl * 32 + ch * 8);
-        }
-        __syncthreads();
+        const int ep_cg = tid & 3;
+        int voff_r[3];
+#pragma unroll
+        for (int q = 0; q < 3; ++q) voff_r[q] = tid + 512 * q < NPIX * 4 ? (((tid + 512 * q) >> 2) * C + ep_cg * 8) * 2 : (int)OOB;
+        u32x4 r0[3], r1[3];
+        f32x4 b0[2], b1[2];
+#define S4_FETCH(pass, R, B)                                                                                              \
+        {                                                                                                                  \
+            _Pragma("unroll") for (int q = 0; q < 3; ++q) R[q] = __builtin_amdgcn_raw_buffer_load_b128(rs_x, voff_r[q], (pass) * 64, 0); \
+            B[0] = *reinterpret_cast<const f32x4*>(a.b_up + (pass) * 32 + ep_cg * 8);                                      \
+            B[1] = *reinterpret_cast<const f32x4*>(a.b_up + (pass) * 32 + ep_cg * 8 + 4);                                  \
+        }
+#define S4_PASS(pass, RC, BC, RN, BN, next)                                                                               \
+        {                                                                                                                  \
+            S4_FETCH(next, RN, BN)                                                                                         \
+            f32x4 acc[3][2];                                                                                               \
+            _Pragma("unroll") for (int i = 0; i < 3; ++i)                                                                  \
+                _Pragma("unroll") for (int j = 0; j < 2; ++j) acc[i][j] = f32x4{0.f, 0.f, 0.f, 0.f};                       \
+            _Pragma("unroll") for (int sl = 0; sl < 3; ++sl) {                                                             \
+                vec8 fb[2];                                                                                                \
+                _Pragma("unroll") for (int j = 0; j < 2; ++j)                                                              \
+                    fb[j] = *reinterpret_cast<const vec8*>(sStage + swz64(sl * 256 + (pass) * 32 + j * 16 + fr, fq));      \
+                _Pragma("unroll") for (int i = 0; i < 3; ++i)                                                              \
+                    if (i < nfr) {                                                                                         \
+                        const vec8 fa = *reinterpret_cast<const vec8*>(sMixed + sl * SLICE_BYTES + swz64(prow[i], fq));    \
+                        _Pragma("unroll") for (int j = 0; j < 2; ++j) acc[i][j] = LP<T>::mfma(fb[j], fa, acc[i][j]);       \
+                    }                                                                                                      \
+            }                                                                                                              \
+            FN_PH(14)                                                                                                      \
+            _Pragma("unroll") for (int i = 0; i < 3; ++i)                                                                  \
+                if (i < nfr) {                                                                                             \
+                    _Pragma("unroll") for (int j = 0; j < 2; ++j)                                                          \
+                        *reinterpret_cast<f32x4*>(&sC[prow[i] * CLD + j * 16 + fq * 4]) = acc[i][j];                       \
+                }                                                                                                          \
+            __syncthreads();                                                                                               \
+            FN_PH(15)                                                                                                      \
+            FN_PH_WAIT(7)          \
+            FN_PH(16)                                                                                                      \
+            _Pragma("unroll") for (int q = 0; q < 3; ++q)                                                                  \
+                if (tid + 512 * q < NPIX * 4) {                                                                            \
+                    const int pp = (tid + 512 * q) >> 2, col = (pass) * 32 + ep_cg * 8;                                    \
+                    const f32x4 c0 = *reinterpret_cast<const f32x4*>(&sC[pp * CLD + ep_cg * 8]);                           \
+                    const f32x4 c1 = *reinterpret_cast<const f32x4*>(&sC[pp * CLD + ep_cg * 8 + 4]);                       \
+                    float rv[8], v[8];                                                                                     \
+                    unpack8<T>(RC[q], rv);                                                                                 \
+                    _Pragma("unroll") for (int e = 0; e < 4; ++e) {                                                        \
+                        v[e] = rv[e] + a.scale * (c0[e] + BC[0][e]);                                                       \
+                        v[4 + e] = rv[4 + e] + a.scale * (c1[e] + BC[1][e]);                                               \
+                    }                                                                                                      \
+                    if (a.relu) {                                                                                          \
+                        _Pragma("unroll") for (int e = 0; e < 8; ++e) v[e] = fmaxf(v[e], 0.f);                             \
+                    }                                                                                                      \
+                    *reinterpret_cast<u32x4*>(a.y + ((long)img * NPIX + pp) * C + col) = pack8<T>(v);                      \
+                }                                                                                                          \
+            __syncthreads();                                                                                               \
+            FN_PH(17)                                                                                                      \
+        }
+        S4_FETCH(0, r0, b0)
+        FN_PH(13)
 #pragma unroll 1
-        for (int pass = 0; pass < 8; ++pass) {
-            f32x4 acc[3][2];
-#pragma unroll
-            for (int i = 0; i < 3; ++i)
-#pragma unroll
-                for (int j = 0; j < 2; ++j) acc[i][j] = f32x4{0.f, 0.f, 0.f, 0.f};
-#pragma unroll
-            for (int sl = 0; sl < 3; ++sl) {
-                vec8 fb[2];
-#pragma unroll
-                for (int j = 0; j < 2; ++j) fb[j] = *reinterpret_cast<const vec8*>(sStage + swz64(sl * 256 + pass * 32 + j * 16 + fr, fq));
-#pragma unroll
-                for (int i = 0; i < 3; ++i)
-                    if (i < nfr) {
-                        const vec8 fa = *reinterpret_cast<const vec8*>(sMixed + sl * SLICE_BYTES + swz64(prow[i], fq));
-#pragma unroll
-                        for (int j = 0; j < 2; ++j) acc[i][j] = LP<T>::mfma(fa, fb[j], acc[i][j]);
-                    }
-            }
-#pragma unroll
-            for (int i = 0; i < 3; ++i)
-                if (i < nfr) {
-#pragma unroll
-                    for (int j = 0; j < 2; ++j)
-#pragma unroll
-                        for (int r = 0; r < 4; ++r) sC[((wave + 8 * i) * 16 + fq * 4 + r) * CLD + j * 16 + fr] = acc[i][j][r];
-                }
-            __syncthreads();
-            for (int idx = tid; idx < NPIX * 4; idx += 512) {
-                const int p = idx >> 2, cg = idx & 3;
-                const int col = pass * 32 + cg * 8;
-                const f32x4 c0 = *reinterpret_cast<const f32x4*>(&sC[p * CLD + cg * 8]);
-                const f32x4 c1 = *reinterpret_cast<const f32x4*>(&sC[p * CLD + cg * 8 + 4]);
-                const f32x4 b0 = *reinterpret_cast<const f32x4*>(a.b_up + col), b1 = *reinterpret_cast<const f32x4*>(a.b_up + col + 4);
-                float rv[8], v[8];
-                unpack8<T>(load_global_b128(xin, (long)p * C + col), rv);
-#pragma unroll
-                for (int e = 0; e < 4; ++e) {
-                    v[e] = rv[e] + a.scale * (c0[e] + b0[e]);
-                    v[4 + e] = rv[4 + e] + a.scale * (c1[e] + b1[e]);
-                }
-                if (a.relu) {
-#pragma unroll
-                    for (int e = 0; e < 8; ++e) v[e] = fmaxf(v[e], 0.f);
-                }
-                *reinterpret_cast<u32x4*>(a.y + ((long)img * NPIX + p) * C + col) = pack8<T>(v);
-            }
-            __syncthreads();
-        }
+        for (int pass = 0; pass < 8; pass += 2) {
+            S4_PASS(pass, r0, b0, r1, b1, pass + 1)
+            S4_PASS(pass + 1, r1, b1, r0, b0, min(pass + 2, 7))
+        }
+#undef S4_FETCH
+#undef S4_PASS
     }
 }
 
@@ -655,7 +750,8 @@
                   (const unsigned short*)w_t1b, (const unsigned short*)w_t1c, (const unsigned short*)w_up, b_t0, b_t1a, b_t1b, b_t1c, b_up,
                   scale, relu, N, (const unsigned char*)warm, (long)warm_bytes};
     const int grid = N + (warm ? WARM_WGS : 0);
-    constexpr size_t smem = 8 * 64 * 64 + 2 * 4 * 112 * 64 + 3 * 16 * 1024;
+    constexpr size_t smem = 8 * 64 * 64 + 2 * 4 * 112 * 64 + 3 * 20 * 1024;
+    static_assert(smem <= 160 * 1024 && 64 * 132 * 4 <= 2 * 4 * 112 * 64, "block17 LDS plan: mixed 32 KB | two patches 56 KB (fp32 C tile over them) | staging 60 KB");
     static const int use_dma = env_int("FN_B17_DMA", 1);
     static LdsOptIn ok[4];
     const void* kerns[4] = {reinterpret_cast<const void*>(block17_infer_kernel<__bf16, false>), reinterpret_cast<const void*>(block17_infer_kernel<_Float16, false>),
```
